# mdolab/adflow

Measured on AMD Instinct MI355X. Metric: Mcells*residual-evals/s, higher is better.
Workload: dtype f64

## Files before the change

adflow_amd/csrc/api.hip:

```cpp
#include <hip/hip_runtime.h>

#include <algorithm>
#include <cmath>
#include <cstdarg>
#include <cstdio>
#include <cstring>
#include <functional>
#include <map>
#include <string>
#include <tuple>
#include <vector>

#include "internal.h"
#include "flow_plan.h"

extern int g_march_kch, g_viscous_tiled, g_inviscid_march, g_roe_march, g_sa_march;
int g_test_fault = 0;
int g_rvec_joint = 1;
int g_pc_fused = 1;
int g_xcd_tiles = 2;

namespace {

std::string g_err;
int g_device = -1;
hipStream_t g_stream = nullptr;
hipStream_t g_streamB = nullptr, g_streamC = nullptr;
hipEvent_t g_evFork = nullptr, g_evB = nullptr, g_evC = nullptr, g_evB1 = nullptr;
hipStream_t g_streamX = nullptr;
hipEvent_t g_evPack = nullptr, g_evComm = nullptr;
int g_overlap = 1;
adflow_opts g_opts;
bool g_have_opts = false;
hipEvent_t g_events[64];
bool g_events_ready = false;
bool g_async = false;

int fail(const char* fmt, ...)
{
    char buf[1024];
    va_list ap;
    va_start(ap, fmt);
    vsnprintf(buf, sizeof buf, fmt, ap);
    va_end(ap);
    g_err = buf;
    return 1;
}

#define HIPCHK(expr)                                                                        \
    do {                                                                                    \
        hipError_t e_ = (expr);                                                             \
        if (e_ != hipSuccess) return fail("%s failed: %s (%s:%d)", #expr, hipGetErrorString(e_), __FILE__, __LINE__); \
    } while (0)

struct DevArr {
    double* base = nullptr;
    int ncomp = 0;
};

struct Block {
    adflow_block_desc d;
    BlkView v;
    long boxsize = 0;
    std::vector<void*> allocs;
    bool geom_uploaded = false;
    bool normals_from_x_ok = true;
    unsigned geom_is_host = 0;
    bool face_vectors_valid = false;
    bool ss_valid = false;
    bool etot_consistent = false;
    std::vector<BcFaceDev> bc;
    std::vector<void*> bc_allocs;
    int nViscBocos = 0;
    double *wref = nullptr, *dwref = nullptr, *jac = nullptr, *snap = nullptr;
    void *jac_raw = nullptr, *snap_raw = nullptr;
    int jac_ncomp = 0, snap_ncomp = 0;
    int* wd_ind = nullptr;
    double* wd_uv = nullptr;
    int wd_max_node = 0;
};

typedef std::tuple<int, int, int> Key;
std::map<Key, Block*> g_blocks;

// ... 831 lines not shown
}

int adflow_gpu_upload_array(int nn, int level, int sps, int which, const double* host)
{
    Block* b = find_block(nn, level, sps);
    if (!b) return fail("block (%d,%d,%d) not registered", nn, level, sps);
    if (!host) return fail("null host pointer");
    double* dev; int nc, lo[3], n[3];
    if (array_spec(b, which, &dev, &nc, lo, n)) return 1;
    if (copy_box(b, dev, host, nc, lo[0], n[0], lo[1], n[1], lo[2], n[2], true)) return 1;
    if (which == ADFLOW_ARR_W || which == ADFLOW_ARR_P || which == ADFLOW_ARR_GAMMA) {
        b->ss_valid = false;
        b->etot_consistent = false;
    }
    if (which == ADFLOW_ARR_X || which == ADFLOW_ARR_SI || which == ADFLOW_ARR_SJ || which == ADFLOW_ARR_SK) {
        if (sync_and_check()) return 1;
        b->face_vectors_valid = false;
        const double* own = which == ADFLOW_ARR_X ? b->d.x : which == ADFLOW_ARR_SI ? b->d.sI : which == ADFLOW_ARR_SJ ? b->d.sJ : b->d.sK;
        const unsigned bit = which == ADFLOW_ARR_X ? 1u : which == ADFLOW_ARR_SI ? 2u : which == ADFLOW_ARR_SJ ? 4u : 8u;
        if (host == own) b->geom_is_host |= bit; else b->geom_is_host &= ~bit;
        b->normals_from_x_ok = b->geom_is_host == 15 && normals_match_nodes(b);
    }
    return sync_and_check();
}

int adflow_gpu_time_step(int level, int onlyRadii)
{
    if (need_ready()) return 1;
    KParams kp = make_kparams(level, 1.0, 0);
    kp.onlyRadii = onlyRadii;
    if (time_step_level(level, kp)) return 1;
    return sync_and_check();
}

int adflow_gpu_initres(int level, int varStart, int varEnd)
{
    if (need_ready()) return 1;
    if (varEnd < varStart) return 0;
    KParams kp = make_kparams(level, 1.0, 0);
    int rc = for_level(level, [&](Block* b) {
        if (varStart < 1 || varEnd > b->v.nw) return fail("initres: variable range %d..%d outside 1..%d", varStart, varEnd, b->v.nw);
        return 0;
    });
    if (rc) return rc;
    LevelTab t;
    if (level_tab(level, &t)) return 1;
    launch_initres_level(t.tab, t.n, t.nx, t.ny, t.nz, kp, varStart - 1, varEnd - 1, g_stream);
    return sync_and_check();
}

static int enqueue_flow_fluxes(int level, const KParams& kp, const struct FlowPlan& P, bool needGrad);
static int source_terms_enqueue(int withBlank);

static int wall_stress_enqueue(int level, const KParams& kp, bool formGrad);

static bool has_wall_subfaces(int level);

static bool level_at_rest(int level)
{
    bool anyMoving = false;
    for_level(level, [&](Block* b) { anyMoving = anyMoving || b->v.sFace || b->v.moving; return 0; });
    return !anyMoving;
}

static void block_face_vectors(Block* b)
{
    if (b->face_vectors_valid) return;
    launch_face_vectors(b->v, g_stream);
    b->face_vectors_valid = true;
}
static int ensure_face_vectors(int level)
{
    return for_level(level, [&](Block* b) { block_face_vectors(b); return 0; });
}

static KParams res_kparams(int level, unsigned flags)
{
    KParams kp = make_kparams(level, 1.0, 0);
    kp.onlyRadii = !(flags & ADFLOW_RES_UPDATE_INTERMED);
    kp.coarseInit = 0;
    if (level == 1 && g_rvec_target) { kp.rvec = g_rvec_target; kp.rvecTurbScale = g_opts.turbResScale; }
    kp.dissApprox = (flags & ADFLOW_RES_DISS_APPROX) ? 1 : 0;
    if (kp.dissApprox && (flags & ADFLOW_RES_UPWIND_FIRST_ORDER)) kp.lumpedDiss = 1;
    return kp;
}

static FlowFacts flow_facts(int level, const KParams& kp, bool viscApprox, bool needGradHbm, bool dual = false,
                            unsigned resFlags = ADFLOW_RES_FLOW)
{
    FlowFacts f = {};
    f.spaceDiscr = kp.spaceDiscr; f.viscous = kp.viscous; f.fineGrid = kp.fineGrid; f.fwMode = kp.fwMode; f.dissApprox = kp.dissApprox;
    f.lumpedDiss = kp.lumpedDiss; f.limiter = kp.limiter; f.coarseInit = kp.coarseInit; f.onlyRadii = kp.onlyRadii;
    f.doScaling = kp.doScaling; f.rvec = kp.rvec != nullptr; f.rFil = kp.rFil; f.adis = kp.adis;
    f.viscApprox = viscApprox; f.needGradHbm = needGradHbm; f.dual = dual;
    f.wantFlow = (resFlags & ADFLOW_RES_FLOW) != 0; f.wantTurb = (resFlags & ADFLOW_RES_TURB) != 0;
    f.atRest = level_at_rest(level);
    f.rans = g_opts.equations == ADFLOW_RANS;
    f.eulerMarch = g_use_march; f.inviscidMarch = g_inviscid_march; f.roeMarch = g_roe_march; f.viscousTiled = g_viscous_tiled;
    f.saMarch = g_sa_march; f.pcFused = g_pc_fused; f.rvecJoint = g_rvec_joint; f.jacSnap = g_jac_snap;
    return f;
}

static int enqueue_flow_residual(int level, const KParams& kp, bool viscApprox = false, bool lowSpeed = true, bool stage0 = true,
                                 bool needGradHbm = false)
{
    const bool wallStress = stage0 && !viscApprox && kp.viscous && level == g_opts.groundLevel && fabs(kp.rFil) >= 1.e-10 &&
                            has_wall_subfaces(level);
    const FlowPlan P = plan_flow(flow_facts(level, kp, viscApprox, needGradHbm));
    if (enqueue_flow_fluxes(level, kp, P, needGradHbm)) return 1;
    if (wallStress)
        if (wall_stress_enqueue(level, kp, P.wallGradOnChip)) return 1;
    if (lowSpeed && level == 1 && source_terms_enqueue(1)) return 1;
    if (lowSpeed && g_opts.lowSpeedPreconditioner) {
        LevelTab t;
        if (level_tab(level, &t)) return 1;
        launch_low_speed_precond_level(t.tab, t.n, t.nx, t.ny, t.nz, kp, g_stream);
    }
    return 0;
}

static int enqueue_flow_fluxes(int level, const KParams& kp, const FlowPlan& P, bool needGrad)
{
    if (kp.spaceDiscr != ADFLOW_DISS_SCALAR && kp.spaceDiscr != ADFLOW_DISS_MATRIX && kp.spaceDiscr != ADFLOW_UPWIND)
        return fail("spaceDiscr=%d not supported (1 scalar, 2 matrix, 9 upwind)", kp.spaceDiscr);
    int nStale = 0, nBlk = 0;
    int rc = for_level(level, [&](Block* b) {
        if (!b->geom_uploaded) return fail("geometry of a level-%d block has not been uploaded", level);
        ++nBlk;
        if (P.needSensor && !b->ss_valid) ++nStale;
        return 0;
    });
    if (rc) return rc;
    if (nStale > 0) {
        if (nStale == nBlk) {
            LevelTab ts;
            if (level_tab(level, &ts)) return 1;
            launch_entropy_level(ts.tab, ts.n, ts.nx, ts.ny, ts.nz, g_stream);
        }
        for_level(level, [&](Block* b) {
            if (nStale != nBlk && !b->ss_valid) launch_entropy(b->v, g_stream);
            b->ss_valid = true;
            return 0;
        });
    }
    LevelTab t;
    if (level_tab(level, &t)) return 1;
    if ((P.needGfTiles && ensure_gf_tiles(level)) || (P.needTiles && ensure_tiles(level))) return 1;
    KParams kv = kp;
    kv.viscFirst = P.viscFirst ? 1 : 0;
    auto inviscid = [&]() -> int {
        switch (P.inviscid) {
        case InviscidK::EulerMarch: launch_euler_march(g_tab[level], g_tiles[level].first, g_tiles[level].second, kv, g_stream); return 0;
        case InviscidK::RoeMarch: return launch_roe_march(g_tab[level], g_tiles[level].first, g_tiles[level].second, kv, g_stream);
        case InviscidK::FaceMarch: return launch_inviscid_march(g_tab[level], g_tiles[level].first, g_tiles[level].second, kv, g_stream);
        case InviscidK::PcMarch: launch_pc_march(g_tab[level], g_tiles[level].first, g_tiles[level].second, kv, g_march_kch, g_stream); return 0;
        case InviscidK::LevelGather: launch_inviscid_level(t.tab, t.n, t.nx, t.ny, t.nz, kv, g_stream); return 0;
        case InviscidK::None: break;
        }
        return 0;
    };
    auto viscous = [&]() -> int {
        switch (P.viscous) {
        case ViscousK::GfMarch: launch_visc_gf(g_tab[level], g_gf_tiles[level].first, g_gf_tiles[level].second, kv, needGrad, g_stream); return 0;
        case ViscousK::ThinLayerMarch: launch_visc_march_approx(g_tab[level], g_tiles[level].first, g_tiles[level].second, kv, g_stream); return 0;
// ... 1472 lines not shown
{
    if (turbBC && apply_turb_bc_enqueue(level, secondHalo)) return 1;
    return apply_bc_enqueue(level, secondHalo);
}

static int apply_bc_enqueue(int level, int secondHalo)
{
    BcPlan* pl;
    if (bc_plan(level, &pl)) return 1;
    if (pl->nent == 0) return 0;
    KParams kp = make_kparams(level, 1.0, 0);
    if (pl->anyEulerWall && g_opts.eulerWallBCTreatment == ADFLOW_WALLBC_QUADRATIC)
        return fail("eulerWallBCTreatment=%d: bcEulerWall has no quadratic extrapolation (1 constant, 2 linear, 4 normal momentum)",
                    g_opts.eulerWallBCTreatment);
    if (pl->anyEulerWall && g_opts.eulerWallBCTreatment == ADFLOW_WALLBC_NORMAL_MOMENTUM && kp.fineGrid) {
        if (!level_at_rest(level))
            return fail("eulerWallBCTreatment = normal momentum on moving blocks needs the cell-centre grid velocity (not mirrored)");
    }
    LevelTab t;
    if (level_tab(level, &t)) return 1;
    launch_apply_all_bc(t.tab, pl->d_ent, pl->d_order, pl->flow, kp, secondHalo, g_opts.eulerWallBCTreatment,
                        g_opts.viscWallBCTreatment, g_opts.outflowTreatment, g_opts.hScalingInlet, g_stream);
    return for_level(level, [&](Block* b) {
        if (!b->bc.empty()) b->ss_valid = false;
        return 0;
    });
}

static int ad_apply_bc_enqueue(int level, const KParams& kp, bool turbBC)
{
    BcPlan* pl;
    if (bc_plan(level, &pl)) return 1;
    if (pl->nent == 0) return 0;
    if (pl->anyEulerWall && g_opts.eulerWallBCTreatment == ADFLOW_WALLBC_QUADRATIC)
        return fail("eulerWallBCTreatment=%d: bcEulerWall has no quadratic extrapolation", g_opts.eulerWallBCTreatment);
    LevelTab t;
    if (level_tab(level, &t)) return 1;
    if (turbBC) ad_launch_turb_bc(g_ad_tab, t.n, pl->maxFace, pl->d_ent, pl->d_order, pl->ordinal, kp, 1, g_stream);
    std::vector<BcPhase> flow;
    for (const BcPhase& ph : pl->flow)
        if (ph.kind != BCP_EXTRAP && ph.kind != BCP_SUPERSONIC_INFLOW) flow.push_back(ph);
    ad_launch_apply_all_bc(g_ad_tab, pl->d_ent, pl->d_order, flow, kp, 1, g_opts.eulerWallBCTreatment, g_opts.viscWallBCTreatment,
                           g_opts.outflowTreatment, g_opts.hScalingInlet, g_stream);
    return 0;
}

static bool has_wall_subfaces(int level)
{
    BcPlan* pl;
    if (bc_plan(level, &pl)) return false;
    return pl->wall.count > 0;
}

static int wall_stress_enqueue(int level, const KParams& kp, bool formGrad)
{
    BcPlan* pl;
    if (bc_plan(level, &pl)) return 1;
    if (pl->wall.count == 0) return 0;
    LevelTab t;
    if (level_tab(level, &t)) return 1;
    launch_wall_stress(t.tab, pl->d_ent, pl->d_order, pl->wall, kp, formGrad, g_stream);
    return 0;
}

int adflow_gpu_download_wall_stress(int nn, int level, int sps, int mm, double* tau, double* q)
{
    Block* b = find_block(nn, level, sps);
    if (!b) return fail("block (%d,%d,%d) not registered", nn, level, sps);
    if (mm < 1 || mm > b->nViscBocos || mm > (int)b->bc.size()) return fail("download_wall_stress: subface %d is not a viscous subface of block %d", mm, nn);
    const BcFaceDev& f = b->bc[mm - 1];
    int r[4];
    bc_owned_range(f.faceID, f.icBeg, f.icEnd, f.jcBeg, f.jcEnd, b->v.il, b->v.jl, b->v.kl, r);
    const long no = (long)std::max(0, r[1] - r[0] + 1) * std::max(0, r[3] - r[2] + 1);
    if (no == 0 || !f.tauq) return 0;
    HIPCHK(hipStreamSynchronize(g_stream));
    if (tau) HIPCHK(hipMemcpy(tau, f.tauq, sizeof(double) * 6 * no, hipMemcpyDeviceToHost));
    if (q) HIPCHK(hipMemcpy(q, f.tauq + 6 * no, sizeof(double) * 3 * no, hipMemcpyDeviceToHost));
    return 0;
}

static int bc_coarse_corrections_enqueue(int coarseLevel, double fact)
{
    BcPlan* pl;
    if (bc_plan(coarseLevel, &pl)) return 1;
    if (pl->nent == 0) return 0;
    LevelTab t;
    if (level_tab(coarseLevel, &t)) return 1;
    launch_bc_coarse_corrections(t.tab, pl->d_ent, pl->d_order, pl->ordinal, fact, g_stream);
    return 0;
}

int adflow_gpu_apply_all_bc(int level, int secondHalo)
{
    if (need_ready()) return 1;
    if (apply_bc_enqueue(level, secondHalo)) return 1;
    return sync_and_check();
}

int adflow_gpu_comm_unique_id(void* id128)
{
#ifndef ADFLOW_NO_RCCL
    if (!id128) return fail("null id buffer");
    ncclUniqueId id;
    NCCLCHK(ncclGetUniqueId(&id));
    memcpy(id128, &id, sizeof id);
    return 0;
#else
    (void)id128;
    return fail("built without RCCL");
#endif
}

int adflow_gpu_comm_init(int rank, int nranks, const void* id128)
{
// ... 513 lines not shown

void set_block_flags(const std::vector<unsigned char>& f)
{
    size_t q = 0;
    for (auto& kv : g_blocks) {
        if (q >= f.size()) break;
        Block* b = kv.second;
        const unsigned char v = f[q++];
        b->geom_uploaded = v & 1; b->normals_from_x_ok = (v >> 1) & 1; b->face_vectors_valid = (v >> 2) & 1; b->ss_valid = (v >> 3) & 1;
        b->etot_consistent = (v >> 4) & 1;
    }
}

bool mg_graph_eligible()
{
#ifdef HOSTSIM
    return false;
#else
    if (!g_mg_graph || g_mgg.failed || g_bc_callback || g_turb_bc_callback || g_phase_base > 0 || !g_act.empty()) return false;
    for (auto& kv : g_comm)
        if (!kv.second.h_sendProc.empty() || !kv.second.h_recvProc.empty() || g_comm_self) return false;
    return true;
#endif
}
}

static int mg_cycle_enqueue(const int32_t* cycling, int nSteps);

int adflow_gpu_mg_cycle(const int32_t* cycling, int nSteps)
{
    if (need_ready()) return 1;
    if (!cycling || nSteps < 1) return fail("mg_cycle: empty cycling strategy");
#ifndef HOSTSIM
    if (mg_graph_eligible()) {
        const bool same = (g_mgg.gen == g_state_gen && (int)g_mgg.cyc.size() == nSteps && !memcmp(g_mgg.cyc.data(), cycling, sizeof(int32_t) * nSteps));
        if (!same) {
            mg_graph_drop();
            g_mgg.cyc.assign(cycling, cycling + nSteps);
            g_mgg.gen = g_state_gen;
        }
        if (g_mgg.exec && block_flags() == g_mgg.pre) {
            HIPCHK(hipGraphLaunch(g_mgg.exec, g_stream));
            set_block_flags(g_mgg.post);
            return sync_and_check();
        }
        if (g_mgg.exec) {
            g_mgg.seen = 0;
        } else if (g_mgg.seen >= 1) {
            HIPCHK(hipStreamSynchronize(g_stream));
            g_mgg.pre = block_flags();
            if (hipStreamBeginCapture(g_stream, hipStreamCaptureModeThreadLocal) == hipSuccess) {
                const bool was = g_async;
                g_async = true;
                const int rc = mg_cycle_enqueue(cycling, nSteps);
                g_async = was;
                hipGraph_t gr = nullptr;
                const hipError_t e1 = hipStreamEndCapture(g_stream, &gr);
                if (rc == 0 && e1 == hipSuccess && gr && !(g_test_fault & 1) && hipGraphInstantiate(&g_mgg.exec, gr, nullptr, nullptr, 0) == hipSuccess) {
                    g_mgg.graph = gr;
                    g_mgg.post = block_flags();
                    HIPCHK(hipGraphLaunch(g_mgg.exec, g_stream));
                    return sync_and_check();
                }
                if (gr) (void)hipGraphDestroy(gr);
                (void)hipGetLastError();
                g_mgg.exec = nullptr;
                g_mgg.failed = true;
                set_block_flags(g_mgg.pre);
            } else {
                (void)hipGetLastError();
                g_mgg.failed = true;
            }
        }
        ++g_mgg.seen;
    }
#endif
    const bool was_async = g_async;
    g_async = true;
    const int rc = mg_cycle_enqueue(cycling, nSteps);
    g_async = was_async;
    if (rc) return rc;
    return sync_and_check();
}

static int mg_cycle_enqueue(const int32_t* cycling, int nSteps)
{
    int level = g_opts.groundLevel;
    int rc = 0;
    for (int n = 0; n < nSteps && !rc; ++n) {
        switch (cycling[n]) {
        case -1:
            level -= 1;
            rc = transfer_to_fine_enqueue(level);
            break;
        case 0: {
            if (n > 0 && cycling[n - 1] != 1) {
                int fwMode;
                const double rFil = rfil_stage0(&fwMode);
                KParams kp = make_kparams(level, rFil, fwMode);
                rc = time_step_level(level, kp);
                if (!rc) rc = enqueue_flow_residual(level, kp);
            }
            if (!rc) rc = (g_opts.smoother == ADFLOW_RUNGE_KUTTA) ? adflow_gpu_rk_smooth(level) : adflow_gpu_dadi_smooth(level);
            break;
        }
        case 1:
            rc = transfer_to_coarse_enqueue(level);
// ... 1447 lines not shown
```

adflow_amd/csrc/kernels_bc.hip:

```cpp
#include <algorithm>
#include <vector>

#include "internal.h"

#define BC_ARGS const BlkView* __restrict__ tab, const BcEntry* __restrict__ ent, const int* __restrict__ order
#define BC_PROLOGUE                                   \
    const BcEntry& e_ = ent[order[blockIdx.y]];       \
    const BlkView& b = tab[e_.slot];                  \
    const BcFaceDev& f = e_.f;

struct BcSlab {
    long c0, c1, c2, c3;
    long f;
    long fn;
};

__device__ __forceinline__ bool bc_slab_t(const BlkView& b, const BcFaceDev& f, long t, BcSlab& s)
{
    const int isize = f.icEnd - f.icBeg + 1, jsize = f.jcEnd - f.jcBeg + 1;
    if (t >= (long)isize * jsize) return false;
    const int i = f.icBeg + (int)(t % isize), j = f.jcBeg + (int)(t / isize);
    long base, step;
    switch (f.faceID) {
    case ADFLOW_IMIN: base = b.idx(0, i, j); step = 1; break;
    case ADFLOW_IMAX: base = b.idx(b.ib, i, j); step = -1; break;
    case ADFLOW_JMIN: base = b.idx(i, 0, j); step = b.ldi; break;
    case ADFLOW_JMAX: base = b.idx(i, b.jb, j); step = -(long)b.ldi; break;
    case ADFLOW_KMIN: base = b.idx(i, j, 0); step = b.ldk; break;
    default: base = b.idx(i, j, b.kb); step = -(long)b.ldk; break;
    }
    s.c0 = base; s.c1 = base + step; s.c2 = base + 2 * step; s.c3 = base + 3 * step;
    s.f = t;
    s.fn = (long)isize * jsize;
    return true;
}
__device__ __forceinline__ bool bc_slab(const BlkView& b, const BcFaceDev& f, BcSlab& s)
{
    return bc_slab_t(b, f, (long)blockIdx.x * blockDim.x + threadIdx.x, s);
}

__device__ __forceinline__ void bc_etot(const BlkView& b, const KParams& kp, long c)
{
    const long nb = b.nbox;
    const double ovgm1 = 1.0 / (kp.gammaConstant - 1.0);
    const double u = b.w[c + nb], v = b.w[c + 2 * nb], w = b.w[c + 3 * nb];
    b.w[c + 4 * nb] = ovgm1 * b.p[c] + 0.5 * b.w[c] * (u * u + v * v + w * w);
}

__device__ __forceinline__ void bc_second_halo(const BlkView& b, const KParams& kp, const BcSlab& s)
{
    const long nb = b.nbox;
    const double factor = 0.5;
    double r = 2.0 * b.w[s.c1] - b.w[s.c2];
    r = fmax(factor * b.w[s.c1], r);
    b.w[s.c0] = r;
#pragma unroll
    for (int l = 1; l <= 3; ++l) b.w[s.c0 + l * nb] = 2.0 * b.w[s.c1 + l * nb] - b.w[s.c2 + l * nb];
    b.p[s.c0] = fmax(factor * b.p[s.c1], 2.0 * b.p[s.c1] - b.p[s.c2]);
    if (kp.viscous) b.rlv[s.c0] = b.rlv[s.c1];
    if (kp.eddyModel) b.rev[s.c0] = b.rev[s.c1];
    bc_etot(b, kp, s.c0);
}

struct BcState { double rho, u, v, w, p, rlv, rev; };
__device__ __forceinline__ void bc_store_halos(const BlkView& b, const KParams& kp, const BcSlab& s, const BcState& h, const BcState& i2,
                                               bool second)
{
    const long nb = b.nbox;
    const double ovgm1 = 1.0 / (kp.gammaConstant - 1.0);
    b.w[s.c1] = h.rho; b.w[s.c1 + nb] = h.u; b.w[s.c1 + 2 * nb] = h.v; b.w[s.c1 + 3 * nb] = h.w;
    b.p[s.c1] = h.p;
    if (kp.viscous) b.rlv[s.c1] = h.rlv;
    if (kp.eddyModel) b.rev[s.c1] = h.rev;
    b.w[s.c1 + 4 * nb] = ovgm1 * h.p + 0.5 * h.rho * (h.u * h.u + h.v * h.v + h.w * h.w);
    if (!second) return;
    const double factor = 0.5;
    const double r0 = fmax(factor * h.rho, 2.0 * h.rho - i2.rho);
    const double u0 = 2.0 * h.u - i2.u, v0 = 2.0 * h.v - i2.v, w0 = 2.0 * h.w - i2.w;
    const double p0 = fmax(factor * h.p, 2.0 * h.p - i2.p);
    b.w[s.c0] = r0; b.w[s.c0 + nb] = u0; b.w[s.c0 + 2 * nb] = v0; b.w[s.c0 + 3 * nb] = w0;
    b.p[s.c0] = p0;
    if (kp.viscous) b.rlv[s.c0] = h.rlv;
    if (kp.eddyModel) b.rev[s.c0] = h.rev;
    b.w[s.c0 + 4 * nb] = ovgm1 * p0 + 0.5 * r0 * (u0 * u0 + v0 * v0 + w0 * w0);
}

__device__ __forceinline__ void bcc_symm(const BlkView& b, const BcFaceDev& f, const BcSlab& s, const KParams& kp, int second)
{
    const long nb = b.nbox;
    const long ch = second ? s.c0 : s.c1, cd = second ? s.c3 : s.c2;
    const double nx = f.norm[s.f], ny = f.norm[s.f + s.fn], nz = f.norm[s.f + 2 * s.fn];
// ... 137 lines not shown
        b.w[s.c1] = rho;
        b.w[s.c1 + nb] = velx;
        b.w[s.c1 + 2 * nb] = vely;
        b.w[s.c1 + 3 * nb] = velz;
    }
    if (kp.viscous) b.rlv[s.c1] = b.rlv[s.c2];
    if (kp.eddyModel) b.rev[s.c1] = b.rev[s.c2];
    bc_etot(b, kp, s.c1);
    if (second) bc_second_halo(b, kp, s);
}
__global__ __launch_bounds__(256) void k_bc_subsonic_inflow(BC_ARGS, KParams kp, int second, int hScalingInlet)
{
    BC_PROLOGUE
    BcSlab s;
    if (!bc_slab(b, f, s)) return;
    bcc_subsonic_inflow(b, f, s, kp, second, hScalingInlet);
}

template <bool ISO>
__device__ __forceinline__ void bcc_nswall(const BlkView& b, const BcFaceDev& f, const BcSlab& s, const KParams& kp, int second, int wallTreatment)
{
    const long nb = b.nbox;
    const double rhok = 0.0;
    BcState i2, h;
    i2.rho = b.w[s.c2]; i2.u = b.w[s.c2 + nb]; i2.v = b.w[s.c2 + 2 * nb]; i2.w = b.w[s.c2 + 3 * nb]; i2.p = b.p[s.c2];
    if (wallTreatment == ADFLOW_WALLBC_CONSTANT) {
        h.p = i2.p - 4.0 * (1.0 / 3.0) * rhok;
    } else {
        h.p = 2 * i2.p - b.p[s.c3];
        if (h.p <= 0.0) h.p = i2.p;
    }
    if (ISO) {
        const double tw = f.tns[s.f];
        const double t2 = i2.p / (kp.RGas * i2.rho);
        double t1 = 2.0 * tw - t2;
        t1 = fmax(0.5 * tw, t1);
        t1 = fmin(2.0 * tw, t1);
        h.rho = h.p / (kp.RGas * t1);
    } else {
        h.rho = i2.rho;
    }
    const double us0 = f.uslip ? f.uslip[s.f] : 0.0, us1 = f.uslip ? f.uslip[s.f + s.fn] : 0.0, us2 = f.uslip ? f.uslip[s.f + 2 * s.fn] : 0.0;
    h.u = -i2.u + 2.0 * us0; h.v = -i2.v + 2.0 * us1; h.w = -i2.w + 2.0 * us2;
    h.rlv = b.rlv[s.c2];
    h.rev = kp.eddyModel ? -b.rev[s.c2] : 0.0;
    bc_store_halos(b, kp, s, h, i2, second != 0);
}
template <bool ISO>
__global__ __launch_bounds__(256) void k_bc_nswall(BC_ARGS, KParams kp, int second, int wallTreatment)
{
    BC_PROLOGUE
    BcSlab s;
    if (!bc_slab(b, f, s)) return;
    bcc_nswall<ISO>(b, f, s, kp, second, wallTreatment);
}

__device__ __forceinline__ double bc_mydim(double x, double y) { return fmax(x - y, 0.0); }

__device__ __forceinline__ void bcc_eulerwall(const BlkView& b, const BcFaceDev& f, const BcSlab& s, const KParams& kp, int second, int wallTreatment)
{
    const long nb = b.nbox;
    double grad = 0.0;
    if (wallTreatment == ADFLOW_WALLBC_LINEAR) grad = b.p[s.c3] - b.p[s.c2];
    const double nx = f.norm[s.f], ny = f.norm[s.f + s.fn], nz = f.norm[s.f + 2 * s.fn];
    const double rface = f.rface ? f.rface[s.f] : 0.0;
    const double u = b.w[s.c2 + nb], v = b.w[s.c2 + 2 * nb], w = b.w[s.c2 + 3 * nb];
    if (wallTreatment == ADFLOW_WALLBC_NORMAL_MOMENTUM) {
        const int isize = f.icEnd - f.icBeg + 1;
        const int a = f.icBeg + (int)(s.f % isize), q = f.jcBeg + (int)(s.f / isize);
        long sa, sb;
        const adf_real8 *Sn, *Sa, *Sb;
        switch (f.faceID) {
        case ADFLOW_IMIN: case ADFLOW_IMAX: sa = b.ldi; sb = b.ldk; Sn = b.sI; Sa = b.sJ; Sb = b.sK; break;
        case ADFLOW_JMIN: case ADFLOW_JMAX: sa = 1; sb = b.ldk; Sn = b.sJ; Sa = b.sI; Sb = b.sK; break;
        default: sa = 1; sb = b.ldi; Sn = b.sK; Sa = b.sI; Sb = b.sJ; break;
        }
        const long cf = (f.faceID == ADFLOW_IMIN || f.faceID == ADFLOW_JMIN || f.faceID == ADFLOW_KMIN) ? s.c1 : s.c2;
        const int am1 = (a - 1 > f.icBeg) ? a - 1 : f.icBeg, ap1 = (a + 1 < f.icEnd) ? a + 1 : f.icEnd;
        const int qm1 = (q - 1 > f.jcBeg) ? q - 1 : f.jcBeg, qp1 = (q + 1 < f.jcEnd) ? q + 1 : f.jcEnd;
        const double a1 = 1.0 / (double)((ap1 - am1 > 1) ? ap1 - am1 : 1), b1 = 1.0 / (double)((qp1 - qm1 > 1) ? qp1 - qm1 : 1);
        const double sixa = 2.0 * Sn[cf], siya = 2.0 * Sn[cf + nb], siza = 2.0 * Sn[cf + 2 * nb];
        const double sjxa = Sa[s.c2 - sa] + Sa[s.c2], sjya = Sa[s.c2 - sa + nb] + Sa[s.c2 + nb],
                     sjza = Sa[s.c2 - sa + 2 * nb] + Sa[s.c2 + 2 * nb];
        const double skxa = Sb[s.c2 - sb] + Sb[s.c2], skya = Sb[s.c2 - sb + nb] + Sb[s.c2 + nb],
                     skza = Sb[s.c2 - sb + 2 * nb] + Sb[s.c2 + 2 * nb];
        const long fjp = s.f + (ap1 - a), fjm = s.f + (am1 - a), fkp = s.f + (long)(qp1 - q) * isize, fkm = s.f + (long)(qm1 - q) * isize;
        const double rxj = a1 * (f.norm[fjp] - f.norm[fjm]), ryj = a1 * (f.norm[fjp + s.fn] - f.norm[fjm + s.fn]),
                     rzj = a1 * (f.norm[fjp + 2 * s.fn] - f.norm[fjm + 2 * s.fn]);
        const double dpj = a1 * (b.p[s.c2 + (ap1 - a) * sa] - b.p[s.c2 + (am1 - a) * sa]);
        const double rxk = b1 * (f.norm[fkp] - f.norm[fkm]), ryk = b1 * (f.norm[fkp + s.fn] - f.norm[fkm + s.fn]),
                     rzk = b1 * (f.norm[fkp + 2 * s.fn] - f.norm[fkm + 2 * s.fn]);
        const double dpk = b1 * (b.p[s.c2 + (qp1 - q) * sb] - b.p[s.c2 + (qm1 - q) * sb]);
        const double ri = nx * sixa + ny * siya + nz * siza;
        const double rj = nx * sjxa + ny * sjya + nz * sjza;
        const double rk = nx * skxa + ny * skya + nz * skza;
        const double qj = u * sjxa + v * sjya + w * sjza;
        const double qk = u * skxa + v * skya + w * skza;
        grad = ((qj * (u * rxj + v * ryj + w * rzj) + qk * (u * rxk + v * ryk + w * rzk)) * b.w[s.c2] - rj * dpj - rk * dpk) / ri;
    }
    b.p[s.c1] = bc_mydim(b.p[s.c2], grad);
    const double vn = 2.0 * (rface - u * nx - v * ny - w * nz);
    b.w[s.c1] = b.w[s.c2];
    b.w[s.c1 + nb] = u + vn * nx;
    b.w[s.c1 + 2 * nb] = v + vn * ny;
    b.w[s.c1 + 3 * nb] = w + vn * nz;
    if (kp.viscous) b.rlv[s.c1] = b.rlv[s.c2];
    if (kp.eddyModel) b.rev[s.c1] = b.rev[s.c2];
// ... 10 lines not shown

__device__ __forceinline__ void bcc_farfield(const BlkView& b, const BcFaceDev& f, const BcSlab& s, const KParams& kp, int second)
{
    const long nb = b.nbox;
    const double gm1 = kp.gammaInf - 1.0;
    const double ovgm1 = 1.0 / gm1;
    const double r0 = 1.0 / kp.wInf[0];
    const double u0 = kp.wInf[1], v0 = kp.wInf[2], w0 = kp.wInf[3];
    const double c0 = sqrt(kp.gammaInf * kp.pInfCorr * r0);
    const double s0 = pow(kp.wInf[0], kp.gammaInf) / kp.pInfCorr;
    const double nx = f.norm[s.f], ny = f.norm[s.f + s.fn], nz = f.norm[s.f + 2 * s.fn];
    const double rface = f.rface ? f.rface[s.f] : 0.0;
    const double qn0 = u0 * nx + v0 * ny + w0 * nz;
    const double vn0 = qn0 - rface;
    const double rho2 = b.w[s.c2], gam2 = b.gamma[s.c2], p2 = b.p[s.c2];
    const double re = 1.0 / rho2;
    const double ue = b.w[s.c2 + nb], ve = b.w[s.c2 + 2 * nb], we = b.w[s.c2 + 3 * nb];
    const double qne = ue * nx + ve * ny + we * nz;
    const double ce = sqrt(gam2 * p2 * re);
    double ac1, ac2;
    if (vn0 > -c0) ac1 = qne + 2.0 * ovgm1 * ce;
    else ac1 = qn0 + 2.0 * ovgm1 * c0;
    if (vn0 > c0) ac2 = qne - 2.0 * ovgm1 * ce;
    else ac2 = qn0 - 2.0 * ovgm1 * c0;
    const double qnf = 0.5 * (ac1 + ac2);
    const double cf = 0.25 * (ac1 - ac2) * gm1;
    double uf, vf, wf, sf;
    if (vn0 > 0.0) {
        uf = ue + (qnf - qne) * nx;
        vf = ve + (qnf - qne) * ny;
        wf = we + (qnf - qne) * nz;
        sf = pow(rho2, gam2) / p2;
    } else {
        uf = u0 + (qnf - qn0) * nx;
        vf = v0 + (qnf - qn0) * ny;
        wf = w0 + (qnf - qn0) * nz;
        sf = s0;
    }
    const double cc = cf * cf / gam2;
    BcState h, i2;
    h.rho = pow(sf * cc, ovgm1);
    h.u = uf; h.v = vf; h.w = wf;
    h.p = h.rho * cc;
    h.rlv = kp.viscous ? b.rlv[s.c2] : 0.0;
    h.rev = kp.eddyModel ? b.rev[s.c2] : 0.0;
    i2.rho = rho2; i2.u = ue; i2.v = ve; i2.w = we; i2.p = p2;
    bc_store_halos(b, kp, s, h, i2, second != 0);
}
__global__ __launch_bounds__(256) void k_bc_farfield(BC_ARGS, KParams kp, int second)
{
    BC_PROLOGUE
    BcSlab s;
    if (!bc_slab(b, f, s)) return;
    bcc_farfield(b, f, s, kp, second);
}

__device__ __forceinline__ void bcc_extrap(const BlkView& b, const BcFaceDev& f, const BcSlab& s, const KParams& kp, int second, int outflowTreatment)
{
    double fw2 = 2.0, fw3 = -1.0;
    if (f.type == ADFLOW_BC_SUPERSONIC_OUTFLOW && outflowTreatment == 1) { fw2 = 1.0; fw3 = 0.0; }
    const long nb = b.nbox;
    const double factor = 0.5;
    BcState h, i2;
    i2.rho = b.w[s.c2]; i2.u = b.w[s.c2 + nb]; i2.v = b.w[s.c2 + 2 * nb]; i2.w = b.w[s.c2 + 3 * nb]; i2.p = b.p[s.c2];
    h.rho = fmax(factor * i2.rho, fw2 * i2.rho + fw3 * b.w[s.c3]);
    h.u = fw2 * i2.u + fw3 * b.w[s.c3 + nb];
    h.v = fw2 * i2.v + fw3 * b.w[s.c3 + 2 * nb];
    h.w = fw2 * i2.w + fw3 * b.w[s.c3 + 3 * nb];
    h.p = fmax(factor * i2.p, fw2 * i2.p + fw3 * b.p[s.c3]);
    h.rlv = kp.viscous ? b.rlv[s.c2] : 0.0;
    h.rev = kp.eddyModel ? b.rev[s.c2] : 0.0;
    bc_store_halos(b, kp, s, h, i2, second != 0);
}
__global__ __launch_bounds__(256) void k_bc_extrap(BC_ARGS, KParams kp, int second, int outflowTreatment)
{
    BC_PROLOGUE
    BcSlab s;
    if (!bc_slab(b, f, s)) return;
    bcc_extrap(b, f, s, kp, second, outflowTreatment);
}

__device__ __forceinline__ void bcc_supersonic_inflow(const BlkView& b, const BcFaceDev& f, const BcSlab& s, const KParams& kp, int second)
{
    const long nb = b.nbox;
    b.w[s.c1] = f.rho[s.f];
    b.w[s.c1 + nb] = f.vx[s.f];
    b.w[s.c1 + 2 * nb] = f.vy[s.f];
    b.w[s.c1 + 3 * nb] = f.vz[s.f];
    b.p[s.c1] = f.ps[s.f];
    if (kp.viscous) b.rlv[s.c1] = b.rlv[s.c2];
    if (kp.eddyModel) b.rev[s.c1] = b.rev[s.c2];
    bc_etot(b, kp, s.c1);
    if (second) {
        b.w[s.c0] = b.w[s.c1];
        b.w[s.c0 + nb] = b.w[s.c1 + nb];
        b.w[s.c0 + 2 * nb] = b.w[s.c1 + 2 * nb];
        b.w[s.c0 + 3 * nb] = b.w[s.c1 + 3 * nb];
        b.p[s.c0] = b.p[s.c1];
        if (kp.viscous) b.rlv[s.c0] = b.rlv[s.c1];
        if (kp.eddyModel) b.rev[s.c0] = b.rev[s.c1];
        bc_etot(b, kp, s.c0);
    }
}
__global__ __launch_bounds__(256) void k_bc_supersonic_inflow(BC_ARGS, KParams kp, int second)
{
    BC_PROLOGUE
    BcSlab s;
// ... 69 lines not shown
    case ADFLOW_BC_SYMM: case ADFLOW_BC_SYMM_POLAR: case ADFLOW_BC_EULERWALL:
        b.bmt[fi][e] = -1.0;
        break;
#ifndef ADF_AD_BUILD
    case ADFLOW_BC_SUPERSONIC_OUTFLOW: case ADFLOW_BC_EXTRAP: case ADFLOW_BC_SUBSONIC_OUTFLOW: case ADFLOW_BC_MASSBLEED_OUTFLOW:
        b.bmt[fi][e] = -1.0;
        break;
    case ADFLOW_BC_SUPERSONIC_INFLOW: case ADFLOW_BC_SUBSONIC_INFLOW:
        if (f.turbInlet) {
            b.bvt[fi][e] = 2.0 * f.turbInlet[t];
            b.bmt[fi][e] = 1.0;
        }
        break;
#endif
    case ADFLOW_BC_FARFIELD: {
        const double dot = f.norm[t] * kp.wInf[1] + f.norm[t + n] * kp.wInf[2] + f.norm[t + 2 * n] * kp.wInf[3] -
                           (f.rface ? f.rface[t] : 0.0);
        if (dot > 0.0) b.bmt[fi][e] = -1.0;
        else b.bvt[fi][e] = kp.wInf[5];
        break;
    }
    default: break;
    }
}
__global__ __launch_bounds__(256) void k_turb_bc_treatment(BC_ARGS, KParams kp)
{
    BC_PROLOGUE
    const long t = (long)blockIdx.x * blockDim.x + threadIdx.x;
    const long n = (long)(f.icEnd - f.icBeg + 1) * (f.jcEnd - f.jcBeg + 1);
    if (t >= n || !b.bmt[0]) return;
    bcc_turb_treatment(b, f, t, kp);
}

__device__ __forceinline__ void bcc_turb_apply(const BlkView& b, const BcFaceDev& f, const BcSlab& s, const KParams& kp, int second)
{
    int fi;
    const long e = bc_face_entry(b, f, s.f, &fi);
    const long nt = 5 * b.nbox;
    b.w[s.c1 + nt] = b.bvt[fi][e] - b.bmt[fi][e] * b.w[s.c2 + nt];
    if (kp.eddyModel) {
        const bool wall = (f.type == ADFLOW_BC_NSWALL_ADIABATIC || f.type == ADFLOW_BC_NSWALL_ISOTHERMAL);
        b.rev[s.c1] = wall ? -b.rev[s.c2] : b.rev[s.c2];
    }
    if (second) {
        b.w[s.c0 + nt] = b.w[s.c1 + nt];
        if (kp.eddyModel) b.rev[s.c0] = b.rev[s.c1];
    }
}
__global__ __launch_bounds__(256) void k_apply_turb_bc(BC_ARGS, KParams kp, int second)
{
    BC_PROLOGUE
    BcSlab s;
    if (!bc_slab(b, f, s) || !b.bmt[0]) return;
    bcc_turb_apply(b, f, s, kp, second);
}


void launch_turb_bc_treatment(const BlkView* tab, int nslots, long maxFace, const BcEntry* ent, const int* order,
                              const std::vector<BcPhase>& ordinal, const KParams& kp, hipStream_t s)
{
    hipLaunchKernelGGL(k_turb_bc_zero, dim3((unsigned)((maxFace + 255) / 256), nslots), dim3(256), 0, s, tab);
    for (const BcPhase& ph : ordinal)
        hipLaunchKernelGGL(k_turb_bc_treatment, bc_grid(ph), dim3(256), 0, s, tab, ent, order + ph.first, kp);
}

void launch_apply_turb_bc(const BlkView* tab, const BcEntry* ent, const int* order, const std::vector<BcPhase>& ordinal,
                          const KParams& kp, int second, hipStream_t s)
{
    for (const BcPhase& ph : ordinal)
        hipLaunchKernelGGL(k_apply_turb_bc, bc_grid(ph), dim3(256), 0, s, tab, ent, order + ph.first, kp, second);
}

__device__ __forceinline__ void crh_copy(const BlkView& b, const KParams& kp, long dst, long src)
{
#pragma unroll
    for (int l = 0; l < 5; ++l) b.w[dst + l * b.nbox] = b.w[src + l * b.nbox];
    b.p[dst] = b.p[src];
    if (kp.viscous) b.rlv[dst] = b.rlv[src];
    if (kp.eddyModel) b.rev[dst] = b.rev[src];
}

__global__ __launch_bounds__(256) void k_corner_row_halos(const BlkView* __restrict__ tab, KParams kp)
{
    const BlkView& b = tab[blockIdx.x + 1];
    if (b.nx == 0) return;
    const int t = threadIdx.x, nt = blockDim.x;
    const int il = b.il, jl = b.jl, kl = b.kl, ie = b.ie, je = b.je, ke = b.ke;
    const int J4[4] = {2, (3 < jl) ? 3 : jl, jl, (2 > b.ny) ? 2 : b.ny};
    const int K4[4] = {2, (3 < kl) ? 3 : kl, kl, (2 > b.nz) ? 2 : b.nz};
    const int I4[4] = {2, (3 < il) ? 3 : il, il, (2 > b.nx) ? 2 : b.nx};
    for (int k = 2 + t; k <= kl; k += nt)
        for (int q = 0; q < 4; ++q) { crh_copy(b, kp, b.idx(1, J4[q], k), b.idx(2, J4[q], k)); crh_copy(b, kp, b.idx(ie, J4[q], k), b.idx(il, J4[q], k)); }
    __syncthreads();
    for (int j = 3 + t; j <= b.ny; j += nt)
        for (int q = 0; q < 4; ++q) { crh_copy(b, kp, b.idx(1, j, K4[q]), b.idx(2, j, K4[q])); crh_copy(b, kp, b.idx(ie, j, K4[q]), b.idx(il, j, K4[q])); }
    __syncthreads();
    for (int k = 3 + t; k <= b.nz; k += nt)
        for (int q = 0; q < 4; ++q) { crh_copy(b, kp, b.idx(I4[q], 1, k), b.idx(I4[q], 2, k)); crh_copy(b, kp, b.idx(I4[q], je, k), b.idx(I4[q], jl, k)); }
    __syncthreads();
    for (int i = 1 + t; i <= ie; i += nt)
        for (int q = 0; q < 4; ++q) { crh_copy(b, kp, b.idx(i, 1, K4[q]), b.idx(i, 2, K4[q])); crh_copy(b, kp, b.idx(i, je, K4[q]), b.idx(i, jl, K4[q])); }
    __syncthreads();
    for (int j = 1 + t; j <= je; j += nt)
        for (int q = 0; q < 4; ++q) { crh_copy(b, kp, b.idx(I4[q], j, 1), b.idx(I4[q], j, 2)); crh_copy(b, kp, b.idx(I4[q], j, ke), b.idx(I4[q], j, kl)); }
    __syncthreads();
    for (int i = 1 + t; i <= ie; i += nt)
        for (int q = 0; q < 4; ++q) { crh_copy(b, kp, b.idx(i, J4[q], 1), b.idx(i, J4[q], 2)); crh_copy(b, kp, b.idx(i, J4[q], ke), b.idx(i, J4[q], kl)); }
// ... 37 lines not shown
```

Measured before the change: 4795.

## Stage i-face BC lines in registers and run wall stress on a side stream

For i-min and i-max boundary faces, the nswall, farfield and turbulence BC kernels now load the four contiguous cells of each variable along i into a small register line, using 16-byte double2 loads when aligned. They run the existing BC body on this local copy and write the halos back with paired stores. This is meant to replace scattered scalar accesses with coalesced vector ones. Separately, the wall-stress kernel is forked onto a secondary stream so it can overlap the flux kernels, except during graph capture. This adds event synchronisation, and the local BlkView remapping relies on the BC bodies only touching the four staged cells.

```diff
diff --git a/adflow_amd/csrc/api.hip b/adflow_amd/csrc/api.hip
--- a/adflow_amd/csrc/api.hip
+++ b/adflow_amd/csrc/api.hip
@@ -30,6 +30,7 @@
 hipStream_t g_streamX = nullptr;
 hipEvent_t g_evPack = nullptr, g_evComm = nullptr;
 int g_overlap = 1;
+bool g_capturing = false;
 adflow_opts g_opts;
 bool g_have_opts = false;
 hipEvent_t g_events[64];
@@ -967,7 +968,7 @@
 static int enqueue_flow_fluxes(int level, const KParams& kp, const struct FlowPlan& P, bool needGrad);
 static int source_terms_enqueue(int withBlank);
 
-static int wall_stress_enqueue(int level, const KParams& kp, bool formGrad);
+static int wall_stress_enqueue(int level, const KParams& kp, bool formGrad, hipStream_t s = nullptr);
 
 static bool has_wall_subfaces(int level);
 
@@ -1022,9 +1023,18 @@
     const bool wallStress = stage0 && !viscApprox && kp.viscous && level == g_opts.groundLevel && fabs(kp.rFil) >= 1.e-10 &&
                             has_wall_subfaces(level);
     const FlowPlan P = plan_flow(flow_facts(level, kp, viscApprox, needGradHbm));
+    const bool wallBeside = wallStress && P.wallGradOnChip && g_overlap && g_streamB && !g_capturing;
+    if (wallBeside) HIPCHK(hipEventRecord(g_evFork, g_stream));
     if (enqueue_flow_fluxes(level, kp, P, needGradHbm)) return 1;
-    if (wallStress)
+    if (wallBeside) {
+        HIPCHK(hipStreamWaitEvent(g_streamB, g_evFork, 0));
+        const int rcw = wall_stress_enqueue(level, kp, true, g_streamB);
+        HIPCHK(hipEventRecord(g_evB, g_streamB));
+        HIPCHK(hipStreamWaitEvent(g_stream, g_evB, 0));
+        if (rcw) return 1;
+    } else if (wallStress) {
         if (wall_stress_enqueue(level, kp, P.wallGradOnChip)) return 1;
+    }
     if (lowSpeed && level == 1 && source_terms_enqueue(1)) return 1;
     if (lowSpeed && g_opts.lowSpeedPreconditioner) {
         LevelTab t;
@@ -2603,14 +2613,14 @@
     return pl->wall.count > 0;
 }
 
-static int wall_stress_enqueue(int level, const KParams& kp, bool formGrad)
+static int wall_stress_enqueue(int level, const KParams& kp, bool formGrad, hipStream_t s)
 {
     BcPlan* pl;
     if (bc_plan(level, &pl)) return 1;
     if (pl->wall.count == 0) return 0;
     LevelTab t;
     if (level_tab(level, &t)) return 1;
-    launch_wall_stress(t.tab, pl->d_ent, pl->d_order, pl->wall, kp, formGrad, g_stream);
+    launch_wall_stress(t.tab, pl->d_ent, pl->d_order, pl->wall, kp, formGrad, s ? s : g_stream);
     return 0;
 }
 
@@ -3230,7 +3240,9 @@
             if (hipStreamBeginCapture(g_stream, hipStreamCaptureModeThreadLocal) == hipSuccess) {
                 const bool was = g_async;
                 g_async = true;
+                g_capturing = true;
                 const int rc = mg_cycle_enqueue(cycling, nSteps);
+                g_capturing = false;
                 g_async = was;
                 hipGraph_t gr = nullptr;
                 const hipError_t e1 = hipStreamEndCapture(g_stream, &gr);
diff --git a/adflow_amd/csrc/kernels_bc.hip b/adflow_amd/csrc/kernels_bc.hip
--- a/adflow_amd/csrc/kernels_bc.hip
+++ b/adflow_amd/csrc/kernels_bc.hip
@@ -37,6 +37,88 @@
 __device__ __forceinline__ bool bc_slab(const BlkView& b, const BcFaceDev& f, BcSlab& s)
 {
     return bc_slab_t(b, f, (long)blockIdx.x * blockDim.x + threadIdx.x, s);
+}
+
+enum { BCL_P = 6, BCL_RLV = 7, BCL_REV = 8, BCL_GAMMA = 9, BCL_NARR = 10 };
+#define BCL_W(l) (1u << (l))
+#define BCL_W14 0xFu
+
+#ifndef ADF_AD_BUILD
+struct BcLine { double v[BCL_NARR][4]; };
+
+__device__ __forceinline__ double* bcl_arr(const BlkView& b, int a)
+{
+    if (a < 6) return b.w + (long)a * b.nbox;
+    if (a == BCL_P) return b.p;
+    if (a == BCL_RLV) return b.rlv;
+    if (a == BCL_REV) return b.rev;
+    return b.gamma;
+}
+__device__ __forceinline__ bool bcl_aligned(const BlkView& b, long base)
+{
+    const uintptr_t any = (uintptr_t)b.w | (uintptr_t)b.p | (uintptr_t)b.rlv | (uintptr_t)b.rev | (uintptr_t)b.gamma;
+    return (any & 15u) == 0 && ((b.nbox | base) & 1) == 0;
+}
+template <bool V16>
+__device__ __forceinline__ void bcl_load2(const double* q, double* d)
+{
+    if (V16) { const double2 t = *reinterpret_cast<const double2*>(q); d[0] = t.x; d[1] = t.y; }
+    else { d[0] = q[0]; d[1] = q[1]; }
+}
+template <bool V16>
+__device__ __forceinline__ void bcl_store2(double* q, const double* d)
+{
+    if (V16) { double2 t; t.x = d[0]; t.y = d[1]; *reinterpret_cast<double2*>(q) = t; }
+    else { q[0] = d[0]; q[1] = d[1]; }
+}
+template <bool MAX, bool V16, class Body>
+__device__ __forceinline__ void bc_line_run(const BlkView& b, const BcFaceDev& f, const BcSlab& s, unsigned rd, unsigned wr, bool second,
+                                            Body body)
+{
+    const long base = MAX ? s.c3 : s.c0;
+    const int ip = MAX ? 0 : 2, hp = MAX ? 2 : 0;
+    BcLine st;
+#pragma unroll
+    for (int a = 0; a < BCL_NARR; ++a)
+        if (rd & (1u << a)) bcl_load2<V16>(bcl_arr(b, a) + base + ip, &st.v[a][ip]);
+    BlkView lb = b;
+    lb.nbox = 4;
+    lb.w = &st.v[0][0]; lb.p = st.v[BCL_P]; lb.rlv = st.v[BCL_RLV]; lb.rev = st.v[BCL_REV]; lb.gamma = st.v[BCL_GAMMA];
+    BcFaceDev lf = f;
+    lf.faceID = MAX ? ADFLOW_IMAX : ADFLOW_IMIN;
+    BcSlab ls = s;
+    ls.c0 = MAX ? 3 : 0; ls.c1 = MAX ? 2 : 1; ls.c2 = MAX ? 1 : 2; ls.c3 = MAX ? 0 : 3;
+    body(lb, lf, ls);
+#pragma unroll
+    for (int a = 0; a < BCL_NARR; ++a)
+        if (wr & (1u << a)) {
+            double* q = bcl_arr(b, a) + base;
+            if (second) bcl_store2<V16>(q + hp, &st.v[a][hp]);
+            else q[ls.c1] = st.v[a][ls.c1];
+        }
+}
+#endif
+
+template <class Body>
+__device__ __forceinline__ void bc_run(const BlkView& b, const BcFaceDev& f, const BcSlab& s, unsigned rd, unsigned wr, bool second, Body body)
+{
+#ifndef ADF_AD_BUILD
+    if (f.faceID == ADFLOW_IMIN) {
+        if (bcl_aligned(b, s.c0)) bc_line_run<false, true>(b, f, s, rd, wr, second, body);
+        else bc_line_run<false, false>(b, f, s, rd, wr, second, body);
+        return;
+    }
+    if (f.faceID == ADFLOW_IMAX) {
+        if (bcl_aligned(b, s.c3)) bc_line_run<true, true>(b, f, s, rd, wr, second, body);
+        else bc_line_run<true, false>(b, f, s, rd, wr, second, body);
+        return;
+    }
+#endif
+    body(b, f, s);
+}
+__device__ __forceinline__ unsigned bcl_halo_set(const KParams& kp)
+{
+    return BCL_W14 | BCL_W(4) | (1u << BCL_P) | (kp.viscous ? 1u << BCL_RLV : 0u) | (kp.eddyModel ? 1u << BCL_REV : 0u);
 }
 
 __device__ __forceinline__ void bc_etot(const BlkView& b, const KParams& kp, long c)
@@ -280,7 +362,9 @@
     BC_PROLOGUE
     BcSlab s;
     if (!bc_slab(b, f, s)) return;
-    bcc_nswall<ISO>(b, f, s, kp, second, wallTreatment);
+    const unsigned rd = BCL_W14 | (1u << BCL_P) | (1u << BCL_RLV) | (kp.eddyModel ? 1u << BCL_REV : 0u);
+    bc_run(b, f, s, rd, bcl_halo_set(kp), second != 0,
+           [&](const BlkView& bb, const BcFaceDev& ff, const BcSlab& ss) { bcc_nswall<ISO>(bb, ff, ss, kp, second, wallTreatment); });
 }
 
 __device__ __forceinline__ double bc_mydim(double x, double y) { return fmax(x - y, 0.0); }
@@ -397,7 +481,9 @@
     BC_PROLOGUE
     BcSlab s;
     if (!bc_slab(b, f, s)) return;
-    bcc_farfield(b, f, s, kp, second);
+    const unsigned rd = BCL_W14 | (1u << BCL_P) | (1u << BCL_GAMMA) | (kp.viscous ? 1u << BCL_RLV : 0u) | (kp.eddyModel ? 1u << BCL_REV : 0u);
+    bc_run(b, f, s, rd, bcl_halo_set(kp), second != 0,
+           [&](const BlkView& bb, const BcFaceDev& ff, const BcSlab& ss) { bcc_farfield(bb, ff, ss, kp, second); });
 }
 
 __device__ __forceinline__ void bcc_extrap(const BlkView& b, const BcFaceDev& f, const BcSlab& s, const KParams& kp, int second, int outflowTreatment)
@@ -573,7 +659,9 @@
     BC_PROLOGUE
     BcSlab s;
     if (!bc_slab(b, f, s) || !b.bmt[0]) return;
-    bcc_turb_apply(b, f, s, kp, second);
+    const unsigned set = BCL_W(5) | (kp.eddyModel ? 1u << BCL_REV : 0u);
+    bc_run(b, f, s, set, set, second != 0,
+           [&](const BlkView& bb, const BcFaceDev& ff, const BcSlab& ss) { bcc_turb_apply(bb, ff, ss, kp, second); });
 }
 
 
```

New measurement: 4799 (median of 2 runs). Within noise of the previous version (+0.1%).
